# mehta-lab/dynamorph

Measured on AMD Instinct MI355X. Metric: cell-patches/sec (128x128x2) VQ-VAE fwd+bwd, higher is better.
Workload: dtype f32; 1 GPU; C3: VQ_VAE training step (forward + backward + fused Adam), 2x128x128 fp32 synthetic patches; per_gpu_batch=2048, global_batch=2048, parallelism=dp1, hip_graph=True, fused_trainer=True, backward_products=f32

## Files before the change

### dynamorph_amd/csrc/convT_bwd.hip

```cpp
#include "dm_common.h"
#include "tile.h"

namespace {

constexpr int CT_TH = 8;

template <int CI, int CO, int TW>
struct ConvTBwdGeom {
    static constexpr int GROWS = 2 * CT_TH + 2, RSG = 2 * TW + 8, C4G = RSG / 4;
    static constexpr int PSG_RAW = GROWS * RSG, PSG = PSG_RAW + ((4 - (PSG_RAW % 32)) + 32) % 32;
    static constexpr int PSS_RAW = CT_TH * TW, PSS = PSS_RAW + ((4 - (PSS_RAW % 32)) + 32) % 32;
    static constexpr int NG4 = CO * GROWS * C4G, NS4 = CI * CT_TH * (TW / 4);
    static constexpr int EG = (NG4 + DM_BLOCK - 1) / DM_BLOCK, ES = (NS4 + DM_BLOCK - 1) / DM_BLOCK;
    static constexpr int TILE_FLOATS = CO * PSG + CI * PSS;
    static constexpr int RED_FLOATS = 4 * CO * 256;
    static constexpr int LDS_FLOATS = TILE_FLOATS > RED_FLOATS ? TILE_FLOATS : RED_FLOATS;
};

constexpr int convT_bwd_wgs(int CI) { return CI == 8 ? 3 : 2; }

template <int CI, int CO, int TW>
__global__ __launch_bounds__(DM_BLOCK, convT_bwd_wgs(CI))
void convT_bwd_kernel(const float *__restrict__ S, const float *__restrict__ G, const float *__restrict__ w,
                      float *__restrict__ gin, double *__restrict__ stats, float *__restrict__ wslabs, int mask_relu, int H,
                      int W, int ntiles)
{
    using Geo = ConvTBwdGeom<CI, CO, TW>;
    static_assert(CI <= 16 && TW % 16 == 0, "one tile of input channels; rows of whole 16-position groups");
    constexpr int GROWS = Geo::GROWS, RSG = Geo::RSG, C4G = Geo::C4G, PSG = Geo::PSG, PSS = Geo::PSS;
    constexpr bool HALF = CI == 8;
    constexpr int EG = Geo::EG, ES = Geo::ES, CG = TW / 16;
    constexpr int MTW = (HALF ? CT_TH / 2 : CT_TH) * CG / 4;
    constexpr int KS = HALF ? CO * 6 : CO * 4;
    constexpr int NWT = HALF ? CO / 2 : CO;
    static_assert(!HALF || CO % 2 == 0, "HALF: (co, py, kx) tiles of 16");
    __shared__ __attribute__((aligned(16))) float lds[Geo::LDS_FLOATS];
    __shared__ double s_stat[4][16];
    float *sG = lds, *sS = lds + CO * PSG;

    const int lane = threadIdx.x & 63, m = lane & 15, kq = lane >> 4;
    const int wave = __builtin_amdgcn_readfirstlane(threadIdx.x >> 6);
    const int OH = 2 * H, OW = 2 * W, tiles_x = W / TW, tiles_y = H / CT_TH;

    float wreg[KS];
#pragma unroll
    for (int s = 0; s < KS; ++s) {
        if constexpr (HALF) {
            const int co = s / 6, ky = s % 6 - 2 * (m >> 3);
            wreg[s] = (ky >= 0 && ky <= 3) ? w[((m & 7) * CO + co) * 16 + ky * 4 + kq] : 0.f;
        } else {
            wreg[s] = m < CI ? w[(m * CO + (s >> 2)) * 16 + (s & 3) * 4 + kq] : 0.f;
        }
    }

    static_assert(Geo::NS4 % DM_BLOCK == 0 && PSG - Geo::PSG_RAW >= 4, "whole passes over S; a float4 of padding behind G's plane 0");
    int g_lds[EG], g_row[EG], g_col[EG], g_ch[EG];
#pragma unroll
    for (int e = 0; e < EG; ++e) {
        const int i = e * DM_BLOCK + threadIdx.x;
        const int co = i / (GROWS * C4G), rem = i - co * (GROWS * C4G), lr = rem / C4G, c4 = rem - lr * C4G;
        g_ch[e] = i < Geo::NG4 ? co : -1;
        g_row[e] = lr; g_col[e] = 4 * c4;
        g_lds[e] = i < Geo::NG4 ? co * PSG + lr * RSG + 4 * c4 : Geo::PSG_RAW;
    }
    int s_lds[ES], s_off[ES];
#pragma unroll
    for (int e = 0; e < ES; ++e) {
        const int i = e * DM_BLOCK + threadIdx.x;
        const int ci = i / (CT_TH * (TW / 4)), rem = i - ci * (CT_TH * (TW / 4)), lr = rem / (TW / 4), c4 = rem - lr * (TW / 4);
        s_lds[e] = ci * PSS + lr * TW + 4 * c4;
        s_off[e] = ((ci * H + lr) * W + 4 * c4) * 4;
    }
    f32x4 rg[EG], rs[ES];
    auto coords = [&](int t, int &b, int &y0, int &x0) {
        x0 = (t % tiles_x) * TW; t /= tiles_x;
        y0 = (t % tiles_y) * CT_TH; b = t / tiles_y;
    };
    auto issue = [&](int t, bool live) {
        int b, y0, x0;
        coords(t, b, y0, x0);
        const __amdgpu_buffer_rsrc_t rG = tile_rsrc(G, (long long)b * CO * OH * OW, CO * OH * OW, live);
        const __amdgpu_buffer_rsrc_t rS = tile_rsrc(S, (long long)b * CI * H * W, CI * H * W, live);
        const int so = (y0 * W + x0) * 4;
#pragma unroll
        for (int e = 0; e < EG; ++e) {
            const int gr = 2 * y0 - 1 + g_row[e], gc = 2 * x0 - 4 + g_col[e];
            const bool ok = g_ch[e] >= 0 && (unsigned)gr < (unsigned)OH && (unsigned)gc < (unsigned)OW;
            rg[e] = tile_load4(rG, ok ? ((g_ch[e] * OH + gr) * OW + gc) * 4 : DM_TILE_VOFF_NONE);
            __builtin_amdgcn_sched_barrier(0);
        }
#pragma unroll
        for (int e = 0; e < ES; ++e) {
            rs[e] = tile_load4(rS, s_off[e] + so);
            __builtin_amdgcn_sched_barrier(0);
        }
    };

    f32x4 wacc[NWT];
#pragma unroll
    for (int t = 0; t < NWT; ++t) wacc[t] = (f32x4){0.f, 0.f, 0.f, 0.f};
    double s1 = 0.0;
    const int wsy = HALF ? (m >> 3) : 0;
    const int wa = HALF ? (m & 7) * PSS + kq - wsy * TW : (m < CI ? m : 0) * PSS + kq;
    const float wa_on = (HALF || m < CI) ? 1.f : 0.f;
    int wbt[NWT];
#pragma unroll
    for (int t = 0; t < NWT; ++t) {
        if constexpr (HALF) {
            const int n = 16 * t + m;
            wbt[t] = (n >> 3) * PSG + ((n >> 2) & 1) * RSG + (n & 3) + 3 + 2 * kq;
        } else {
            wbt[t] = t * PSG + (m >> 2) * RSG + (m & 3) + 3 + 2 * kq;
        }
    }

    auto commit = [&]() {
#pragma unroll
        for (int e = 0; e < EG; ++e) *reinterpret_cast<f32x4 *>(sG + g_lds[e]) = rg[e];
#pragma unroll
        for (int e = 0; e < ES; ++e) *reinterpret_cast<f32x4 *>(sS + s_lds[e]) = rs[e];
    };
    int tile = blockIdx.x;
    const bool any = tile < ntiles;
    issue(tile, any);
    if (any) commit();
    while (any) {
        __syncthreads();
        int b, y0, x0;
        coords(tile, b, y0, x0);
        tile += gridDim.x;
        issue(tile, tile < ntiles);

        if constexpr (HALF) {
            auto steps = [&](int Yr, int s0, int ns) {
                const float on = (Yr - wsy >= 0 && Yr - wsy < CT_TH) ? 1.f : 0.f;
                const float *pa = sS + wa + (on != 0.f ? Yr * TW : wsy * TW);
                for (int s = s0; s < s0 + ns; ++s) {
                    const float a = pa[4 * s] * on;
#pragma unroll
                    for (int t = 0; t < NWT; ++t)
                        wacc[t] = __builtin_amdgcn_mfma_f32_16x16x4f32(a, sG[wbt[t] + 2 * Yr * RSG + 8 * s], wacc[t], 0, 0, 0);
                }
            };
            steps(wave, 0, TW / 4);
            steps(wave + 4, 0, TW / 4);
            steps(CT_TH, wave * (TW / 16), TW / 16);
        } else {
#pragma unroll
            for (int rr = 0; rr < 2; ++rr) {
                const int row = wave + 4 * rr;
                const float *pa = sS + wa + row * TW;
#pragma unroll
                for (int s = 0; s < TW / 4; ++s) {
                    const float a = pa[4 * s] * wa_on;
#pragma unroll
                    for (int t = 0; t < NWT; ++t)
                        wacc[t] = __builtin_amdgcn_mfma_f32_16x16x4f32(a, sG[wbt[t] + 2 * row * RSG + 8 * s], wacc[t], 0, 0, 0);
                }
            }
        }
        float *__restrict__ gb = gin + (long long)b * CI * H * W + (long long)y0 * W + x0;
#pragma unroll
        for (int i = 0; i < MTW; ++i) {
            const int ti = wave + 4 * i, rp = ti / CG, cg = ti - rp * CG;
            f32x4 acc = {0.f, 0.f, 0.f, 0.f};
            const float *pa = sG + (HALF ? 4 : 2) * rp * RSG + 2 * (16 * cg + m) + kq + 3;
#pragma unroll
            for (int s = 0; s < KS; ++s) {
                const int off = HALF ? (s / 6) * PSG + (s % 6) * RSG : (s >> 2) * PSG + (s & 3) * RSG;
                acc = __builtin_amdgcn_mfma_f32_16x16x4f32(pa[off], wreg[s], acc, 0, 0, 0);
            }
            const int ci = HALF ? (m & 7) : m, r = HALF ? 2 * rp + (m >> 3) : rp;
            if (HALF || m < CI) {
                const int off = r * TW + 16 * cg + 4 * kq;
                if (mask_relu) acc = relu_gate4(*reinterpret_cast<const f32x4 *>(sS + ci * PSS + off), acc);
                *reinterpret_cast<f32x4 *>(gb + ((long long)ci * H + r) * W + 16 * cg + 4 * kq) = acc;
                s1 += (double)pair_sum4(acc);
            }
        }
        if (tile >= ntiles) break;
        __syncthreads();
        commit();
    }

    __syncthreads();
    if (stats) stat_fold<16, false, HALF>(&s_stat[0][0], wave, lane, s1);
    float *red = lds;
#pragma unroll
    for (int t = 0; t < NWT; ++t) *reinterpret_cast<f32x4 *>(red + ((wave * NWT + t) * 64 + lane) * 4) = wacc[t];
    __syncthreads();
    if (stats) stat_slab<4, 16, false>(&s_stat[0][0], stats + (long long)blockIdx.x * CI * 2, CI);
    for (int i = threadIdx.x; i < CI * CO * 16; i += DM_BLOCK) {
        const int ci = i / (CO * 16), rem = i - ci * (CO * 16), co = rem >> 4, ky = (rem >> 2) & 3, kx = rem & 3;
        int row, t, n;
        if constexpr (HALF) { row = ci + 8 * (ky >> 1); const int col = co * 8 + (ky & 1) * 4 + kx; t = col >> 4; n = col & 15; }
        else { row = ci; t = co; n = ky * 4 + kx; }
        const int ln = (row >> 2) * 16 + n, r = row & 3;
        float sum = 0.f;
#pragma unroll
        for (int wv = 0; wv < 4; ++wv) sum += red[((wv * NWT + t) * 64 + ln) * 4 + r];
        wslabs[(long long)blockIdx.x * CI * CO * 16 + i] = sum;
    }
}

int convT_bwd_tw(int CI, int CO, int W)
{
    if (CI == 8 && CO == 4) return W % 32 == 0 ? 32 : 0;
    if (CI == 16 && CO == 8) return W % 16 == 0 ? 16 : 0;
    return 0;
}
bool convT_bwd_shape(int CI, int CO, int H, int W) { return H > 0 && W > 0 && H % CT_TH == 0 && convT_bwd_tw(CI, CO, W) > 0; }

}

extern "C" int dm_convt_bwd_fused_supported(int CI, int CO, int H, int W) { return convT_bwd_shape(CI, CO, H, W) ? 1 : 0; }

extern "C" int dm_convt_bwd_fused_num_blocks(int B, int CI, int CO, int H, int W)
{
    if (B <= 0 || !convT_bwd_shape(CI, CO, H, W)) return -1;
    const long long ntiles = (long long)B * (H / CT_TH) * (W / convT_bwd_tw(CI, CO, W));
    const long long cap = 256LL * convT_bwd_wgs(CI);
    return (int)(ntiles < cap ? ntiles : cap);
}

extern "C" int dm_convt_bwd_fused(const float *S, const float *G, const float *w, float *gin, double *stats, float *wslabs,
                                  int mask_relu, int B, int CI, int CO, int H, int W, void *stream)
{
    DM_REQUIRE(S && G && w && gin && wslabs, "dm_convt_bwd_fused: NULL pointer");
    DM_REQUIRE(B > 0 && convT_bwd_shape(CI, CO, H, W), "dm_convt_bwd_fused: ConvTranspose2d(%d -> %d) on %dx%d not built", CI, CO, H, W);
    DM_REQUIRE((long long)B * CO * 4 * H * W < (1LL << 31), "dm_convt_bwd_fused: tensor too large");
    const int ntiles = B * (H / CT_TH) * (W / convT_bwd_tw(CI, CO, W));
    const int grid = dm_convt_bwd_fused_num_blocks(B, CI, CO, H, W);
    hipStream_t st = (hipStream_t)stream;
#define DM_CTB(CI_, CO_, TW_)                                                                                          \
    hipLaunchKernelGGL((convT_bwd_kernel<CI_, CO_, TW_>), dim3(grid), dim3(DM_BLOCK), 0, st, S, G, w, gin, stats, wslabs, \
                       mask_relu, H, W, ntiles)
    if (CI == 8) DM_CTB(8, 4, 32);
    else DM_CTB(16, 8, 16);
#undef DM_CTB
    return dm_launch_status("dm_convt_bwd_fused");
}
```

Before: 1.105 million patches/s.

## Restructure HALF convT backward: shared row products, S halo row, pipelined LDS loads

```diff
diff --git a/dynamorph_amd/csrc/convT_bwd.hip b/dynamorph_amd/csrc/convT_bwd.hip
--- a/dynamorph_amd/csrc/convT_bwd.hip
+++ b/dynamorph_amd/csrc/convT_bwd.hip
@@ -8,9 +8,10 @@
 template <int CI, int CO, int TW>
 struct ConvTBwdGeom {
     static constexpr int GROWS = 2 * CT_TH + 2, RSG = 2 * TW + 8, C4G = RSG / 4;
+    static constexpr int SHALO = CI == 8 ? 1 : 0, SROWS = CT_TH + SHALO;
     static constexpr int PSG_RAW = GROWS * RSG, PSG = PSG_RAW + ((4 - (PSG_RAW % 32)) + 32) % 32;
-    static constexpr int PSS_RAW = CT_TH * TW, PSS = PSS_RAW + ((4 - (PSS_RAW % 32)) + 32) % 32;
-    static constexpr int NG4 = CO * GROWS * C4G, NS4 = CI * CT_TH * (TW / 4);
+    static constexpr int PSS_RAW = SROWS * TW, PSS = PSS_RAW + ((4 - (PSS_RAW % 32)) + 32) % 32;
+    static constexpr int NG4 = CO * GROWS * C4G, NS4 = CI * SROWS * (TW / 4);
     static constexpr int EG = (NG4 + DM_BLOCK - 1) / DM_BLOCK, ES = (NS4 + DM_BLOCK - 1) / DM_BLOCK;
     static constexpr int TILE_FLOATS = CO * PSG + CI * PSS;
     static constexpr int RED_FLOATS = 4 * CO * 256;
@@ -30,10 +31,11 @@
     constexpr int GROWS = Geo::GROWS, RSG = Geo::RSG, C4G = Geo::C4G, PSG = Geo::PSG, PSS = Geo::PSS;
     constexpr bool HALF = CI == 8;
     constexpr int EG = Geo::EG, ES = Geo::ES, CG = TW / 16;
-    constexpr int MTW = (HALF ? CT_TH / 2 : CT_TH) * CG / 4;
-    constexpr int KS = HALF ? CO * 6 : CO * 4;
+    constexpr int MTW = CT_TH * CG / 4;
+    constexpr int KS = HALF ? CO * 2 : CO * 4;
+    constexpr int SHALO = Geo::SHALO, SROWS = Geo::SROWS;
     constexpr int NWT = HALF ? CO / 2 : CO;
-    static_assert(!HALF || CO % 2 == 0, "HALF: (co, py, kx) tiles of 16");
+    static_assert(!HALF || (CO % 2 == 0 && CG == 2), "HALF: (co, py, kx) tiles of 16; a wave per column group and half of the rows");
     __shared__ __attribute__((aligned(16))) float lds[Geo::LDS_FLOATS];
     __shared__ double s_stat[4][16];
     float *sG = lds, *sS = lds + CO * PSG;
@@ -46,30 +48,39 @@
 #pragma unroll
     for (int s = 0; s < KS; ++s) {
         if constexpr (HALF) {
-            const int co = s / 6, ky = s % 6 - 2 * (m >> 3);
-            wreg[s] = (ky >= 0 && ky <= 3) ? w[((m & 7) * CO + co) * 16 + ky * 4 + kq] : 0.f;
+            const int co = s >> 1, ky = (s & 1) + 2 - 2 * (m >> 3);
+            wreg[s] = w[((m & 7) * CO + co) * 16 + ky * 4 + kq];
         } else {
             wreg[s] = m < CI ? w[(m * CO + (s >> 2)) * 16 + (s & 3) * 4 + kq] : 0.f;
         }
     }
 
-    static_assert(Geo::NS4 % DM_BLOCK == 0 && PSG - Geo::PSG_RAW >= 4, "whole passes over S; a float4 of padding behind G's plane 0");
-    int g_lds[EG], g_row[EG], g_col[EG], g_ch[EG];
+    static_assert(PSG - Geo::PSG_RAW >= 4 && PSS - Geo::PSS_RAW >= 4, "a float4 of padding behind plane 0 of G and of S");
+    int g_lds[EG], g_row[HALF ? 1 : EG], g_col[HALF ? 1 : EG], g_ch[HALF ? 1 : EG], g_off[HALF ? EG : 1], g_edge[HALF ? EG : 1];
 #pragma unroll
     for (int e = 0; e < EG; ++e) {
         const int i = e * DM_BLOCK + threadIdx.x;
         const int co = i / (GROWS * C4G), rem = i - co * (GROWS * C4G), lr = rem / C4G, c4 = rem - lr * C4G;
-        g_ch[e] = i < Geo::NG4 ? co : -1;
-        g_row[e] = lr; g_col[e] = 4 * c4;
+        if constexpr (HALF) {
+            g_off[e] = i < Geo::NG4 ? ((co * OH + lr - 1) * OW + 4 * c4 - 4) * 4 : DM_TILE_VOFF_NONE;
+            g_edge[e] = (lr == 0 ? 1 : 0) | (lr == GROWS - 1 ? 2 : 0) | (c4 == 0 ? 4 : 0) | (c4 == C4G - 1 ? 8 : 0);
+            asm volatile("" : "+v"(g_off[e]));
+        } else {
+            g_ch[e] = i < Geo::NG4 ? co : -1;
+            g_row[e] = lr; g_col[e] = 4 * c4;
+        }
         g_lds[e] = i < Geo::NG4 ? co * PSG + lr * RSG + 4 * c4 : Geo::PSG_RAW;
     }
     int s_lds[ES], s_off[ES];
+    bool s_top[ES];
 #pragma unroll
     for (int e = 0; e < ES; ++e) {
         const int i = e * DM_BLOCK + threadIdx.x;
-        const int ci = i / (CT_TH * (TW / 4)), rem = i - ci * (CT_TH * (TW / 4)), lr = rem / (TW / 4), c4 = rem - lr * (TW / 4);
-        s_lds[e] = ci * PSS + lr * TW + 4 * c4;
-        s_off[e] = ((ci * H + lr) * W + 4 * c4) * 4;
+        const int ci = i / (SROWS * (TW / 4)), rem = i - ci * (SROWS * (TW / 4)), lr = rem / (TW / 4), c4 = rem - lr * (TW / 4);
+        const bool have = Geo::NS4 % DM_BLOCK == 0 || i < Geo::NS4;
+        s_lds[e] = have ? ci * PSS + lr * TW + 4 * c4 : Geo::PSS_RAW;
+        s_off[e] = have ? ((ci * H + lr - SHALO) * W + 4 * c4) * 4 : DM_TILE_VOFF_NONE;
+        s_top[e] = SHALO && lr == 0;
     }
     f32x4 rg[EG], rs[ES];
     auto coords = [&](int t, int &b, int &y0, int &x0) {
@@ -81,17 +92,22 @@
         coords(t, b, y0, x0);
         const __amdgpu_buffer_rsrc_t rG = tile_rsrc(G, (long long)b * CO * OH * OW, CO * OH * OW, live);
         const __amdgpu_buffer_rsrc_t rS = tile_rsrc(S, (long long)b * CI * H * W, CI * H * W, live);
-        const int so = (y0 * W + x0) * 4;
+        const int so = (y0 * W + x0) * 4, go = (2 * y0 * OW + 2 * x0) * 4;
+        const int edges = __builtin_amdgcn_readfirstlane((y0 == 0 ? 1 : 0) | (y0 + CT_TH == H ? 2 : 0) | (x0 == 0 ? 4 : 0) | (x0 + TW == W ? 8 : 0));
 #pragma unroll
         for (int e = 0; e < EG; ++e) {
-            const int gr = 2 * y0 - 1 + g_row[e], gc = 2 * x0 - 4 + g_col[e];
-            const bool ok = g_ch[e] >= 0 && (unsigned)gr < (unsigned)OH && (unsigned)gc < (unsigned)OW;
-            rg[e] = tile_load4(rG, ok ? ((g_ch[e] * OH + gr) * OW + gc) * 4 : DM_TILE_VOFF_NONE);
+            if constexpr (HALF) {
+                rg[e] = tile_load4(rG, (g_edge[e] & edges) ? DM_TILE_VOFF_NONE : g_off[e] + go);
+            } else {
+                const int gr = 2 * y0 - 1 + g_row[e], gc = 2 * x0 - 4 + g_col[e];
+                const bool ok = g_ch[e] >= 0 && (unsigned)gr < (unsigned)OH && (unsigned)gc < (unsigned)OW;
+                rg[e] = tile_load4(rG, ok ? ((g_ch[e] * OH + gr) * OW + gc) * 4 : DM_TILE_VOFF_NONE);
+            }
             __builtin_amdgcn_sched_barrier(0);
         }
 #pragma unroll
         for (int e = 0; e < ES; ++e) {
-            rs[e] = tile_load4(rS, s_off[e] + so);
+            rs[e] = tile_load4(rS, (s_top[e] && y0 == 0) ? DM_TILE_VOFF_NONE : s_off[e] + so);
             __builtin_amdgcn_sched_barrier(0);
         }
     };
@@ -101,7 +117,7 @@
     for (int t = 0; t < NWT; ++t) wacc[t] = (f32x4){0.f, 0.f, 0.f, 0.f};
     double s1 = 0.0;
     const int wsy = HALF ? (m >> 3) : 0;
-    const int wa = HALF ? (m & 7) * PSS + kq - wsy * TW : (m < CI ? m : 0) * PSS + kq;
+    const int wa = HALF ? (m & 7) * PSS + kq + (SHALO - wsy) * TW : (m < CI ? m : 0) * PSS + kq;
     const float wa_on = (HALF || m < CI) ? 1.f : 0.f;
     int wbt[NWT];
 #pragma unroll
@@ -132,19 +148,39 @@
         issue(tile, tile < ntiles);
 
         if constexpr (HALF) {
-            auto steps = [&](int Yr, int s0, int ns) {
-                const float on = (Yr - wsy >= 0 && Yr - wsy < CT_TH) ? 1.f : 0.f;
-                const float *pa = sS + wa + (on != 0.f ? Yr * TW : wsy * TW);
+            auto steps = [&](int Yr, int s0, int ns, bool last) {
+                const float *pa = sS + wa + (last ? Yr - 1 + wsy : Yr) * TW;
                 for (int s = s0; s < s0 + ns; ++s) {
-                    const float a = pa[4 * s] * on;
+                    const float a = (last && wsy == 0) ? 0.f : pa[4 * s];
 #pragma unroll
                     for (int t = 0; t < NWT; ++t)
                         wacc[t] = __builtin_amdgcn_mfma_f32_16x16x4f32(a, sG[wbt[t] + 2 * Yr * RSG + 8 * s], wacc[t], 0, 0, 0);
                 }
             };
-            steps(wave, 0, TW / 4);
-            steps(wave + 4, 0, TW / 4);
-            steps(CT_TH, wave * (TW / 16), TW / 16);
+            constexpr int NCH = 2 * TW / 16;
+            float sa[2][4], gb2[2][4][NWT];
+            auto request = [&](int c, int buf) {
+                const int Yr = wave + 4 * (c / (TW / 16)), s0 = 4 * (c % (TW / 16));
+#pragma unroll
+                for (int i = 0; i < 4; ++i) {
+                    sa[buf][i] = sS[wa + Yr * TW + 4 * (s0 + i)];
+#pragma unroll
+                    for (int t = 0; t < NWT; ++t) gb2[buf][i][t] = sG[wbt[t] + 2 * Yr * RSG + 8 * (s0 + i)];
+                }
+            };
+            request(0, 0);
+#pragma unroll
+            for (int c = 0; c < NCH; ++c) {
+                if (c + 1 < NCH) request(c + 1, (c + 1) & 1);
+                __builtin_amdgcn_sched_barrier(0);
+#pragma unroll
+                for (int i = 0; i < 4; ++i)
+#pragma unroll
+                    for (int t = 0; t < NWT; ++t)
+                        wacc[t] = __builtin_amdgcn_mfma_f32_16x16x4f32(sa[c & 1][i], gb2[c & 1][i][t], wacc[t], 0, 0, 0);
+                __builtin_amdgcn_sched_barrier(0);
+            }
+            if (y0 + CT_TH == H) steps(CT_TH, wave * (TW / 16), TW / 16, true);
         } else {
 #pragma unroll
             for (int rr = 0; rr < 2; ++rr) {
@@ -160,22 +196,52 @@
             }
         }
         float *__restrict__ gb = gin + (long long)b * CI * H * W + (long long)y0 * W + x0;
-#pragma unroll
-        for (int i = 0; i < MTW; ++i) {
-            const int ti = wave + 4 * i, rp = ti / CG, cg = ti - rp * CG;
-            f32x4 acc = {0.f, 0.f, 0.f, 0.f};
-            const float *pa = sG + (HALF ? 4 : 2) * rp * RSG + 2 * (16 * cg + m) + kq + 3;
-#pragma unroll
-            for (int s = 0; s < KS; ++s) {
-                const int off = HALF ? (s / 6) * PSG + (s % 6) * RSG : (s >> 2) * PSG + (s & 3) * RSG;
-                acc = __builtin_amdgcn_mfma_f32_16x16x4f32(pa[off], wreg[s], acc, 0, 0, 0);
-            }
-            const int ci = HALF ? (m & 7) : m, r = HALF ? 2 * rp + (m >> 3) : rp;
-            if (HALF || m < CI) {
-                const int off = r * TW + 16 * cg + 4 * kq;
-                if (mask_relu) acc = relu_gate4(*reinterpret_cast<const f32x4 *>(sS + ci * PSS + off), acc);
-                *reinterpret_cast<f32x4 *>(gb + ((long long)ci * H + r) * W + 16 * cg + 4 * kq) = acc;
-                s1 += (double)pair_sum4(acc);
+        auto finish = [&](f32x4 acc, int ci, int r, int cg) {
+            const int off = r * TW + 16 * cg + 4 * kq;
+            if (mask_relu) acc = relu_gate4(*reinterpret_cast<const f32x4 *>(sS + ci * PSS + off + SHALO * TW), acc);
+            *reinterpret_cast<f32x4 *>(gb + ((long long)ci * H + r) * W + 16 * cg + 4 * kq) = acc;
+            s1 += (double)pair_sum4(acc);
+        };
+        if constexpr (HALF) {
+            const int cg = wave & 1, hf = wave >> 1;
+            const float *pa = sG + 8 * hf * RSG + 2 * (16 * cg + m) + kq + 3;
+            f32x4 P[5];
+            float ga[2][KS];
+#pragma unroll
+            for (int s = 0; s < KS; ++s) ga[0][s] = pa[(s >> 1) * PSG + (s & 1) * RSG];
+#pragma unroll
+            for (int u = 0; u < 5; ++u) {
+                if (u + 1 < 5) {
+#pragma unroll
+                    for (int s = 0; s < KS; ++s) ga[(u + 1) & 1][s] = pa[(s >> 1) * PSG + (2 * (u + 1) + (s & 1)) * RSG];
+                }
+                __builtin_amdgcn_sched_barrier(0);
+                P[u] = (f32x4){0.f, 0.f, 0.f, 0.f};
+#pragma unroll
+                for (int s = 0; s < KS; ++s) P[u] = __builtin_amdgcn_mfma_f32_16x16x4f32(ga[u & 1][s], wreg[s], P[u], 0, 0, 0);
+                __builtin_amdgcn_sched_barrier(0);
+            }
+            const bool hi = m >= 8;
+#pragma unroll
+            for (int q = 0; q < 2; ++q) {
+                const f32x4 below = P[2 * q], mid = P[2 * q + 1], above = P[2 * q + 2];
+                f32x4 acc;
+                acc.x = mid.x + lane_xor8(hi ? below.x : above.x);
+                acc.y = mid.y + lane_xor8(hi ? below.y : above.y);
+                acc.z = mid.z + lane_xor8(hi ? below.z : above.z);
+                acc.w = mid.w + lane_xor8(hi ? below.w : above.w);
+                finish(acc, m & 7, 2 * (2 * hf + q) + (m >> 3), cg);
+            }
+        } else {
+#pragma unroll
+            for (int i = 0; i < MTW; ++i) {
+                const int ti = wave + 4 * i, rp = ti / CG, cg = ti - rp * CG;
+                f32x4 acc = {0.f, 0.f, 0.f, 0.f};
+                const float *pa = sG + 2 * rp * RSG + 2 * (16 * cg + m) + kq + 3;
+#pragma unroll
+                for (int s = 0; s < KS; ++s)
+                    acc = __builtin_amdgcn_mfma_f32_16x16x4f32(pa[(s >> 2) * PSG + (s & 3) * RSG], wreg[s], acc, 0, 0, 0);
+                if (m < CI) finish(acc, m, rp, cg);
             }
         }
         if (tile >= ntiles) break;
```

Result: no change. 1.106 million patches/s, median of 4 (+0.0%).
